# V-Sense/LFBM5D

Measured on AMD Instinct MI355X. Metric: SAI-megapixels/sec (HT+Wiener, sigma=25), higher is better.
Workload: dtype f32; 1 GPU; lf17x17x512x512_sigma25; light_field=17x17x512x512x3, asw=1, color_space=opp, noise=MT19937 seed 1 (utilities.cpp:176-183), window_lanes=2, spatial_bands=1, parallelism=single GPU

## Files before the change

### lfbm5d_amd/core.py

```python
import ctypes as C
import os
import subprocess

from typing import NamedTuple, Optional

import numpy as np

_HERE = os.path.dirname(os.path.abspath(__file__))

YUV, YCBCR, OPP, RGB, ID, DCT, SADCT, BIOR, HADAMARD, HAAR = range(10)
ROWMAJOR, COLMAJOR = 11, 12
TAU = {"id": ID, "dct": DCT, "sadct": SADCT, "bior": BIOR, "hw": HADAMARD, "haar": HAAR}
COLOR_SPACE = {"yuv": YUV, "ycbcr": YCBCR, "opp": OPP, "rgb": RGB}
UNIQUE_ID_BYTES = 128


class LfBm5dError(RuntimeError):
    pass


class Params(C.Structure):
    _fields_ = [("sigma", C.c_float), ("lambda_", C.c_float), ("N", C.c_uint), ("nSim", C.c_uint),
                ("nDisp", C.c_uint), ("k", C.c_uint), ("p", C.c_uint), ("useSD", C.c_uint),
                ("tau_2D", C.c_uint), ("tau_4D", C.c_uint), ("tau_5D", C.c_uint),
# ... 224 lines not shown
    import torch
    if not (isinstance(t, torch.Tensor) and t.is_cuda and t.dtype == torch.float32 and t.is_contiguous()):
        raise LfBm5dError("device entry points need contiguous float32 CUDA tensors")
    torch.cuda.current_stream(t.device).synchronize()
    return C.c_void_p(t.data_ptr())


def _sai_ptrs(arrays, mask):
    out = (C.c_void_p * len(arrays))()
    for i, a in enumerate(arrays):
        if a is None or not mask[i]:
            continue
        if not (isinstance(a, np.ndarray) and a.dtype == np.float32 and a.flags.c_contiguous):
            raise LfBm5dError("per-SAI host buffers must be contiguous float32 numpy arrays")
        out[i] = a.ctypes.data
    return out


OPTION_ENV = ("LFBM5D_LANES", "LFBM5D_EMULATE_WORLD", "LFBM5D_MAX_WINDOWS", "LFBM5D_FUSED", "LFBM5D_STEP_SHARDING",
              "LFBM5D_DATA_DRIVEN_SCHEDULE", "LFBM5D_HOST_BLOCKING", "LFBM5D_BAND_MB", "LFBM5D_BM3D_LANES", "LFBM5D_SCAN_LDS_CAP",
              "LFBM5D_FORCE_REDO", "LFBM5D_SPATIAL_BANDS", "LFBM5D_BAND_HALO", "LFBM5D_SCAN_V1", "LFBM5D_SCAN_ANY", "LFBM5D_SCAN_FULL_TABLES", "LFBM5D_DCT8W_V2",
              "LFBM5D_GROUP_GENERIC", "LFBM5D_NO_SA_KERNELS", "LFBM5D_NO_SLAB_KERNEL", "LFBM5D_WIDE_NOSPLIT", "LFBM5D_AGG_64BIT",
              "LFBM5D_AGG_SCALAR_SCAN", "LFBM5D_SUBSET_LIST_HOST", "LFBM5D_SUBSET_SCAN_V1", "LFBM5D_FILT_GROUP_MAJOR",
              "LFBM5D_HT_REF_ORDER")


class Context:

    def __init__(self, device=0):
        self._L = lib()
        h = C.c_void_p()
        if self._L.lfbm5d_create(C.byref(h), int(device)) != 0:
            raise LfBm5dError(self._L.lfbm5d_last_error(None).decode())
        self._handle = h
        self._env_seen = {k: os.environ.get(k) for k in OPTION_ENV}
        self.device = int(device)

    @property
    def _h(self):
        h = self._handle
        if h and hasattr(self._L, "lfbm5d_set_option"):
            for k in OPTION_ENV:
                v = os.environ.get(k)
                if v != self._env_seen[k]:
                    self._env_seen[k] = v
                    self._L.lfbm5d_set_option(h, k.encode(), None if v is None else (v or "1").encode())
        return h

    def set_option(self, key, value):
        if self._L.lfbm5d_set_option(self._handle, key.encode(), None if value is None else str(value).encode()) != 0:
            raise LfBm5dError(self._L.lfbm5d_last_error(self._handle).decode())

    def get_option(self, key):
        buf = C.create_string_buffer(64)
        if self._L.lfbm5d_get_option(self._handle, key.encode(), buf, 64) != 0:
            raise LfBm5dError(self._L.lfbm5d_last_error(self._handle).decode())
        return buf.value.decode()

    def close(self):
        if getattr(self, "_handle", None):
            self._L.lfbm5d_destroy(self._handle)
            self._handle = None

    def __del__(self):
        try:
            self.close()
        except Exception:
            pass
# ... 246 lines not shown
```

### lfbm5d_amd/csrc/lfbm5d_aggregate.hip

```cpp
#include "lfbm5d_kernels.h"

#include <algorithm>
#include <cstdlib>

namespace lfbm5d {

namespace {



constexpr int kAggFlush = 64;
template <bool WINDOWED, int TW, int TH, int kAggPF, int kAggU, bool BIG, bool VEC4>
__global__ __launch_bounds__(64) __attribute__((amdgpu_waves_per_eu((VEC4 && TW == 8 && !BIG) ? 8 : 1))) void k_aggregate(AggArgs a) {
    constexpr int kAggCap = kAggFlush + kAggPF * 64 + kAggU;
    __shared__ uint4 hit_a[kAggCap];
    __shared__ float hit_w2[kAggCap];
    __shared__ float kai[WINDOWED ? 256 : 1];
    const int lane = threadIdx.x;
    const unsigned gx = (a.Wb + TW - 1) / TW, gy = (a.Hb + TH - 1) / TH, total_wg = gx * gy * a.A;
    const unsigned per_xcd = gridDim.x / 8;
    const unsigned lin2 = (blockIdx.x % 8) * per_xcd + blockIdx.x / 8;
    if (lin2 >= total_wg) return;
    const int st = (int)(lin2 / (gx * gy));
    const int tile_y = (int)((lin2 / gx) % gy), tile_x = (int)(lin2 % gx);
    if (a.proc_bits.test((unsigned)st)) return;
    if (!a.mask_bits.test((unsigned)st)) return;
    const int tx0 = tile_x * TW, ty0 = tile_y * TH;
    const int x = tx0 + lane % TW, y = ty0 + lane / TW;
    const bool inside = x < (int)a.Wb && y < (int)a.Hb;
    const int k = a.k, k2 = k * k, C = a.C, N = a.N, A = a.A;
    const int logN = 31 - __builtin_clz((unsigned)N);
    const size_t plane = (size_t)a.Wb * a.Hb;
    const int reach = (st == (int)a.pst) ? (int)a.nSim : (int)a.nHW;
    if (WINDOWED) for (int i = lane; i < k2; i += 64) kai[i] = a.tb->kaiser[i];

    const int last_r = (int)a.Hb - k - (int)a.nHW, last_c = (int)a.Wb - k - (int)a.nHW;
    auto lo_idx = [&](int v) { int d = v - (int)a.nHW; return d <= 0 ? 0 : (d + (int)a.p - 1) / (int)a.p; };
    auto hi_idx = [&](int v, int n, int lastv) {
        if (v >= lastv) return n - 1;
        int d = v - (int)a.nHW; if (d < 0) return -1;
        int i = d / (int)a.p; return i > n - 2 ? n - 2 : i;
    };
    int r_lo = lo_idx(ty0 - k + 1 - reach), r_hi = hi_idx(ty0 + TH - 1 + reach, (int)a.n_ref_rows, last_r);
    int c_lo = lo_idx(tx0 - k + 1 - reach), c_hi = hi_idx(tx0 + TW - 1 + reach, (int)a.n_ref_cols, last_c);
    if (r_lo > (int)a.n_ref_rows - 1) r_lo = (int)a.n_ref_rows - 1;
    if (c_lo > (int)a.n_ref_cols - 1) c_lo = (int)a.n_ref_cols - 1;
    if (!a.irregular && a.n_ref_cols) {
        r_lo = max(r_lo, (int)(a.ref_begin / a.n_ref_cols));
        r_hi = min(r_hi, (int)((a.ref_begin + a.n_groups - 1) / a.n_ref_cols));
    }
    const int ncols_span = c_hi - c_lo + 1;
    const int n_rr = a.irregular ? (int)a.n_groups : ((r_hi >= r_lo && c_hi >= c_lo) ? (r_hi - r_lo + 1) * ncols_span : 0);
    const int n_cand = n_rr << logN;
    if (n_cand == 0) return;

    float accn[3] = {0, 0, 0}, accd[3] = {0, 0, 0};
    const size_t pix = (size_t)st * C * plane + (size_t)y * a.Wb + x;
    if (inside) for (int c = 0; c < C; c++) { accn[c] = a.num[pix + c * plane]; accd[c] = a.den[pix + c * plane]; }

    const bool mul_div = !a.irregular && (long long)n_rr * ncols_span < (1 << 20);
    const unsigned div_m = ((1u << 20) + (unsigned)max(ncols_span, 1) - 1) / (unsigned)max(ncols_span, 1);
    const unsigned g_end = a.ref_begin + a.n_groups;
    const bool sai_major = a.filt_sai_stride != 0;
    const unsigned Af = sai_major ? 1u : (unsigned)A, stf = sai_major ? 0u : (unsigned)st;
    const float* const filt = a.filt + (sai_major ? (size_t)st * a.filt_sai_stride : (size_t)0);
    const unsigned long long filt_bytes = sai_major ? a.filt_sai_stride * sizeof(float) : a.filt_bytes;
    const bool small24 = (((unsigned long long)a.n_refs_total << logN) + 1) * Af < (1ull << 24);
    const unsigned* apos = a.aggpos + (size_t)st * a.n_refs_total * N;
    const unsigned cstride = C > 1 ? (unsigned)k2 * 4u : 0u;
    const __amdgpu_buffer_rsrc_t rs_filt = __builtin_amdgcn_make_buffer_rsrc((void*)filt, 0, BIG ? 0 : (int)(unsigned)filt_bytes, 0x00020000u);
    unsigned nh = 0;

    auto consume = [&]() {
        const unsigned nh_pad = (nh + kAggU - 1) / kAggU * kAggU;
        if (nh + lane < nh_pad) { hit_a[nh + lane] = make_uint4(0xffffffffu, 0u, 0u, 0u); hit_w2[nh + lane] = 0.0f; }
        __builtin_amdgcn_wave_barrier();
        for (unsigned h0 = 0; h0 < nh_pad; h0 += kAggU) {
            float val[kAggU][3], kw[kAggU][3];
#pragma unroll
            for (int u = 0; u < kAggU; u++) {
// ... 136 lines not shown
                const unsigned slot = nh + __popcll(bal & ((1ull << lane) - 1ull));
                unsigned off;
                const unsigned gl = g[u] - a.ref_begin;
                if (small24) off = __umul24(__umul24((gl << logN) + nn[u], Af) + stf, (unsigned)(C * k2));
                else { asm volatile("" ::: "memory"); off = (((gl << logN) + nn[u]) * Af + stf) * C * k2; }
                hit_a[slot] = make_uint4(p[u], off, __float_as_uint(w[u][0]), __float_as_uint(w[u][1]));
                hit_w2[slot] = w[u][2];
            }
            nh += __popcll(bal);
        }
        __builtin_amdgcn_wave_barrier();
        if (nh >= kAggFlush) consume();
    }
    if (nh) consume();
    if (inside) for (int c = 0; c < C; c++) { a.num[pix + c * plane] = accn[c]; a.den[pix + c * plane] = accd[c]; }
}

}

hipError_t launch_aggregate(hipStream_t s, const AggArgs& a) {
    const bool wide = a.k >= 12;
    constexpr int kAgg16TW = 16, kAgg16TH = 4, kAgg8TW = 8, kAgg8TH = 8;
    const unsigned tw = wide ? (a.k == 12 ? 16 : kAgg16TW) : (a.k == 8 ? kAgg8TW : 8), th = wide ? (a.k == 12 ? 4 : kAgg16TH) : (a.k == 8 ? kAgg8TH : 8);
    const unsigned tiles = ((a.Wb + tw - 1) / tw) * ((a.Hb + th - 1) / th) * a.A;
    const dim3 grid(((tiles + 7) / 8) * 8), block(64);
    const bool big = (a.filt_sai_stride ? a.filt_sai_stride * sizeof(float) : a.filt_bytes) > 0xfffff000ull || (a.opt & kOptAgg64Bit);
    const bool vec4 = a.N % 4 == 0 && !wide && !(a.opt & kOptAggScalarScan);
#define LFBM5D_AGG(W_, TW_, TH_, PF_, U_) \
    do { if (big && vec4) hipLaunchKernelGGL((k_aggregate<W_, TW_, TH_, PF_, U_, true, true>), grid, block, 0, s, a); \
         else if (big)    hipLaunchKernelGGL((k_aggregate<W_, TW_, TH_, PF_, U_, true, false>), grid, block, 0, s, a); \
         else if (vec4)   hipLaunchKernelGGL((k_aggregate<W_, TW_, TH_, PF_, U_, false, true>), grid, block, 0, s, a); \
         else             hipLaunchKernelGGL((k_aggregate<W_, TW_, TH_, PF_, U_, false, false>), grid, block, 0, s, a); } while (0)
    constexpr int kAgg16PF = 3, kAgg16U = 12, kAgg8PF = 3, kAgg8U = 6;
    if (a.k == 12)      LFBM5D_AGG(true, 16, 4, 3, 12);
    else if (a.k == 8)  LFBM5D_AGG(true, kAgg8TW, kAgg8TH, kAgg8PF, kAgg8U);
    else if (wide)      LFBM5D_AGG(false, kAgg16TW, kAgg16TH, kAgg16PF, kAgg16U);
    else                LFBM5D_AGG(false, 8, 8, 2, 6);
#undef LFBM5D_AGG
    return hipGetLastError();
}

}
```

### lfbm5d_amd/csrc/lfbm5d_ctx.h

```cpp
#ifndef LFBM5D_CTX_H
#define LFBM5D_CTX_H

#include "../../include/lfbm5d.h"
#include "lfbm5d_kernels.h"
#include "lfbm5d_plan.h"
#include "lfbm5d_options.h"

#include <rccl/rccl.h>

#include <algorithm>
#include <chrono>
#include <cmath>
#include <fstream>
#include <thread>
#include <unistd.h>
#include <cstdio>
#include <cstdlib>
#include <cstring>
#include <string>
#include <vector>


namespace lfbm5d_host {

// ... 44 lines not shown
    float* const* basic = nullptr;
    float* const* out = nullptr;
};

struct lfbm5d_ctx {
    int device = 0;
    hipStream_t stream = nullptr;
    std::string err;
    int rank = 0, world = 1;
    int tiles = 1;
    ncclComm_t comm = nullptr;
    ncclComm_t comm2 = nullptr;
    hipStream_t cs[2] = {nullptr, nullptr};
    int pass_rank = 0, pass_world = 1;
    bool pass_reduce = false;
    std::vector<unsigned> last_windows;
    lfbm5d_stats stats;
    DevBuf t_noisy, t_basic, t_tnum, t_tden, und_num, und_den;
    DevBuf scan_lcol;
    DevBuf sub_flags, sub_cnt;
    int last_scan_version = 0;
    GeomCache gc[2]; int gslot = 0;
    bool est_ready = false;
    DevBuf est, refmap, scores, tables, self_idx, self_cnt, best, shape, filt, wgt, aggpos, gpos, gofs, gok, sa_list, gshape, counters, small, t_num, t_den, d_mask;
    DevBuf g_num, g_den, g_num2, g_den2, n2, e_basic, w_noisy, w_basic, w_num, w_den, h2d_noisy, h2d_basic, h2d_out, d_own, gscratch;
    bool ipc = false;
    std::string ipc_dir; double ipc_timeout_s = 30.0; unsigned ipc_epoch = 0;
    std::string ipc_tag;
    DevBuf ipc_flags, ipc_out;
    struct IpcPeer { unsigned char handle[7][64]; void* ptr[7]; };
    std::vector<IpcPeer> ipc_peers;
    DevBuf pristine, pristine_b;
    DevBuf band_noisy, band_basic, band_out, band_src, band_pack, band_gather;
    ncclComm_t team_comm = nullptr, team_comm2 = nullptr; int team_S = 0;
    Options opt_store; Options* opt = &opt_store;
    hipStream_t io_in = nullptr, io_out = nullptr;
    unsigned* h_small = nullptr;
    struct NoiseBufs { DevBuf sai, part, cells, m, pool; } noise;
    std::vector<lfbm5d_ctx*> lanes;
    unsigned* h_counts = nullptr; size_t h_counts_cap = 0;
    unsigned long long lane_windows = 0;
    std::vector<hipEvent_t> ev_pool; size_t ev_used = 0;
    std::vector<PassEvents> pending;
    unsigned last_n_refs = 0, last_N = 0, last_A = 0; size_t last_plane = 0; int last_gslot = 0;
};

// ... 45 lines not shown
```

### lfbm5d_amd/csrc/lfbm5d_graph.hip

```cpp
#include "lfbm5d_graph.h"

namespace lfbm5d_host {

using plan::search_window;
using plan::plan_windows;

int io_upload_all(lfbm5d_ctx* c, const HostIO* io, const unsigned* h_mask, unsigned asize, size_t img, float* d_noisy, float* d_basic_in) {
    for (unsigned st = 0; st < asize; st++) {
        if (!h_mask[st]) continue;
        HIPCK(c, hipMemcpyAsync(d_noisy + (size_t)st * img, io->noisy[st], img * sizeof(float), hipMemcpyHostToDevice, c->stream));
        if (d_basic_in) HIPCK(c, hipMemcpyAsync(d_basic_in + (size_t)st * img, io->basic[st], img * sizeof(float), hipMemcpyHostToDevice, c->stream));
    }
    HIPCK(c, hipStreamSynchronize(c->stream));
    return 0;
}
int io_download_all(lfbm5d_ctx* c, const HostIO* io, const unsigned* h_mask, unsigned asize, size_t img, const float* d_noisy,
                    const float* d_basic, const float* d_out) {
    for (unsigned st = 0; st < asize; st++) {
        if (!h_mask[st]) continue;
        HIPCK(c, hipMemcpyAsync(io->noisy[st], d_noisy + (size_t)st * img, img * sizeof(float), hipMemcpyDeviceToHost, c->stream));
        if (d_basic) HIPCK(c, hipMemcpyAsync(io->basic[st], d_basic + (size_t)st * img, img * sizeof(float), hipMemcpyDeviceToHost, c->stream));
        if (d_out) HIPCK(c, hipMemcpyAsync(io->out[st], d_out + (size_t)st * img, img * sizeof(float), hipMemcpyDeviceToHost, c->stream));
    }
    HIPCK(c, hipStreamSynchronize(c->stream));
// ... 58 lines not shown


int run_graph(lfbm5d_ctx* c, const GraphJob& J, const plan::Graph& G, const unsigned* h_mask, unsigned awidth, unsigned aheight,
              unsigned ang_major, unsigned W, unsigned H, unsigned C, int nranks, bool emulate, int* complete_out) {
    const unsigned asize = awidth * aheight;
    const size_t img = (size_t)C * W * H;
    hipStream_t s = c->stream;
    const size_t NN = G.nodes.size();
    const bool two = J.n_steps == 2;
    *complete_out = 1;
    struct Geo { unsigned asw, Aw, nHW, wb, hb; size_t imgb; };
    Geo geo[2];
    size_t imgb_max = 0; unsigned Aw_max = 0;
    for (int sl = 0; sl < J.n_steps; sl++) {
        Geo& g = geo[sl];
        g.asw = 2 * J.an[sl] + 1; g.Aw = g.asw * g.asw; g.nHW = J.P[sl]->nSim + J.P[sl]->nDisp;
        g.wb = W + 2 * g.nHW; g.hb = H + 2 * g.nHW; g.imgb = (size_t)C * g.wb * g.hb;
        imgb_max = std::max(imgb_max, g.Aw * g.imgb); Aw_max = std::max(Aw_max, g.Aw);
    }
    const bool any_step2 = J.step[0] == 2 || (two && J.step[1] == 2);

    struct Lane { lfbm5d_ctx* x; float* w_noisy; float* w_basic; float* w_num; float* w_den; unsigned* d_small; };
    struct RankState { int rank; lfbm5d_ctx* x; float* g_num[2]; float* g_den[2]; float* basic; std::vector<Lane> lanes; };
    auto lane_buffers = [&](lfbm5d_ctx* x, Lane& L) -> int {
        HIPCK(c, x->w_noisy.reserve(imgb_max * sizeof(float)));
        if (any_step2) HIPCK(c, x->w_basic.reserve(imgb_max * sizeof(float)));
        HIPCK(c, x->w_num.reserve(imgb_max * sizeof(float)));
        HIPCK(c, x->w_den.reserve(imgb_max * sizeof(float)));
        HIPCK(c, x->small.reserve((asize + 8 + kWinCounters) * sizeof(unsigned)));
        L.x = x; L.w_noisy = x->w_noisy.as<float>(); L.w_basic = x->w_basic.as<float>();
        L.w_num = x->w_num.as<float>(); L.w_den = x->w_den.as<float>(); L.d_small = x->small.as<unsigned>();
        return 0;
    };
    int lanes_used = 1;
    for (const plan::Node& nd : G.nodes) lanes_used = std::max(lanes_used, nd.lane + 1);
    const int lanes_per_rank = emulate ? 1 : lanes_used;
    const size_t need_ctx = emulate ? (size_t)nranks - 1 : (size_t)lanes_used - 1;
    while (c->lanes.size() < need_ctx) {
        std::string e;
        lfbm5d_ctx* x = new_ctx(c->device, e);
        if (!x) return fail(c, "lane context: " + e);
        x->opt = c->opt;
        c->lanes.push_back(x);
    }
    const bool ipc = c->ipc && nranks > 1 && !emulate;
    struct AbortCommsOnError {
        lfbm5d_ctx* c; bool armed;
        ~AbortCommsOnError() {
            if (!armed) return;
            if (c->comm2) { (void)ncclCommAbort(c->comm2); c->comm2 = nullptr; }
            if (c->comm) { (void)ncclCommAbort(c->comm); c->comm = nullptr; }
            (void)hipDeviceSynchronize();
            c->err += " (multi-GPU step aborted: the RCCL communicators of this context were torn down, call lfbm5d_comm_init again)";
        }
// ... 181 lines not shown
            search_window((int)nd.ps, aheight, J.an[sl], cs_w, mins, maxs);
            search_window((int)nd.pt, awidth, J.an[sl], ct_w, mint, maxt);
            const unsigned cst_w = ang_major == LFBM5D_ROWMAJOR ? (unsigned)cs_w * g.asw + (unsigned)ct_w : (unsigned)cs_w + (unsigned)ct_w * g.asw;
            std::vector<unsigned> mask_w(g.Aw, 0), proc_w(g.Aw, 0);
            SaiList wl; wl.n = g.Aw;
            for (unsigned si = 0; si < g.asw; si++)
                for (unsigned ti = 0; ti < g.asw; ti++) {
                    const unsigned Ss = si + (unsigned)mins, T = ti + (unsigned)mint;
                    const unsigned st = ang_major == LFBM5D_ROWMAJOR ? Ss * awidth + T : Ss + T * aheight;
                    const unsigned slot = ang_major == LFBM5D_ROWMAJOR ? si * g.asw + ti : si + ti * g.asw;
                    mask_w[slot] = h_mask[st];
                    wl.st[slot] = h_mask[st] ? st : 0xffffffffu;
                    if (h_mask[st]) win_bits[n].set(slot);
                    proc_w[slot] = !h_mask[st];
                }
            const bool wien = J.step[sl] == 2;
            HIPCK(c, Lw.x->est.reserve((kEstLead + g.Aw * (size_t)g.wb * g.hb + 256) * sizeof(float)));
            HIPCK(c, launch_window_begin(ls, J.noisy[sl], wien ? S->basic : nullptr, S->g_num[sl], S->g_den[sl], img, Lw.w_noisy, Lw.w_basic, Lw.w_num,
                                         Lw.w_den, Lw.x->est.as<float>() + kEstLead, g.imgb, wl, W, H, C, g.nHW, Lw.d_small));
            lfbm5d_params Pw = *J.P[sl];
            Pw.tau_4D = nd.tau4;
            Lw.x->gslot = sl;
            Lw.x->est_ready = true;
            const int prc = pass_impl(Lw.x, J.step[sl], &Pw, g.asw, g.asw, g.wb, g.hb, C, Lw.w_noisy, wien ? Lw.w_basic : nullptr, Lw.w_num, Lw.w_den,
                                      mask_w.data(), proc_w.data(), cst_w, cst_w);
            Lw.x->gslot = 0;
            if (prc) { if (Lw.x != c) c->err = Lw.x->err; return 1; }
            HIPCK(c, launch_window_end(ls, S->g_num[sl], S->g_den[sl], img, Lw.w_num, Lw.w_den, g.imgb, wl, W, H, C, g.nHW, J.P[sl]->k, Lw.d_small));
            HIPCK(c, hipMemcpyAsync(c->h_counts + (size_t)n * kWinCounters, Lw.d_small, kWinCounters * sizeof(unsigned), hipMemcpyDeviceToHost, ls));
            if (!nd.fin.empty()) {
                SaiList fl; fl.n = 0;
                for (unsigned st : nd.fin) fl.st[fl.n++] = st;
                const bool colour = C == 3 && J.P[0]->color_space != LFBM5D_RGB;
                HIPCK(c, launch_finalize_multi(ls, S->g_num[0], S->g_den[0], J.noisy[0], S->basic, img, fl, J.P[0]->color_space, W * H, colour ? 1 : 0));
            }
            done[n] = get_event(c);
            HIPCK(c, hipEventRecord(done[n], ls));
            mine[n] = 1;
            if (io && !outs[n].empty()) {
                for (size_t o0 = 0; o0 < outs[n].size(); o0 += (size_t)kBigA) {
                    SaiList ol; ol.n = 0;
                    for (size_t q = o0; q < outs[n].size() && ol.n < (unsigned)kBigA; q++) ol.st[ol.n++] = outs[n][q];
                    HIPCK(c, launch_output_multi(ls, S->g_num[Ls], S->g_den[Ls], J.step[Ls] == 1 ? J.noisy[Ls] : S->basic, J.d_out,
                                                 J.step[Ls] == 2 ? S->basic : nullptr, J.noisy[Ls], J.d_noisy, img, ol, J.color_space, W * H, colour_io ? 1 : 0));
                }
                ev_out[n] = get_event(c);
// ... 228 lines not shown
```

### lfbm5d_amd/csrc/lfbm5d_kernels.h

```cpp
#ifndef LFBM5D_KERNELS_H
#define LFBM5D_KERNELS_H

#include <hip/hip_runtime.h>
#include <vector>

#include "lfbm5d_options.h"

constexpr int kFiltStoreAux = 2;
constexpr int kFiltLoadAux = 0;

#if defined(__HIPCC__)
typedef float filt_v4f __attribute__((ext_vector_type(4)));
typedef float filt_v2f __attribute__((ext_vector_type(2)));
__device__ __forceinline__ void filt_put(float* p, const float v) { *p = v; }
__device__ __forceinline__ void filt_put2(filt_v2f* p, const filt_v2f v) { *p = v; }
__device__ __forceinline__ void filt_put4(filt_v4f* p, const filt_v4f v) { *p = v; }
__device__ __forceinline__ void filt_put4(float4* p, const float4 v) { *p = v; }
__device__ __forceinline__ void filt_put4_nt(filt_v4f* p, const filt_v4f v) { __builtin_nontemporal_store(v, p); }
#endif

namespace lfbm5d {

constexpr int kMaxK = 32;
constexpr int kMaxA = 49;
// ... 70 lines not shown
    unsigned Wb, Hb, C, A, k, N, pst;
    SaiMask mask_bits, proc_bits;
    unsigned tau2, tau4, tau5, useSD;
    unsigned fill_quirk;
    int step;
    float lambda;
    float sigma[3];
    float ht3_T[3][9][4];
    float ht3_K[3][9];
    float* scratch;
    unsigned long long scratch_floats;
    unsigned opt;
    unsigned long long filt_sai_stride;
    unsigned bm3d;
};

constexpr unsigned kSaiMajorMinA = 121;
__device__ __forceinline__ size_t filt_patch(const GroupArgs& a, unsigned g, unsigned n, unsigned st, unsigned k2) {
    return a.filt_sai_stride ? (size_t)st * a.filt_sai_stride + ((size_t)g * a.N + n) * a.C * k2
                             : (((size_t)g * a.N + n) * a.A + st) * a.C * k2;
}


struct AggArgs {
    float* num;
    float* den;
    const float* filt;
    unsigned long long filt_sai_stride;
    unsigned long long filt_bytes;
    const float* wgt;
    const unsigned* aggpos;
    unsigned n_refs_total;
    const unsigned* refs;
    const unsigned* self_idx;
    const unsigned* self_cnt;
    const unsigned* best;
    const unsigned char* shape;
    const GroupTables* tb;
    unsigned ref_begin, n_groups;
    unsigned n_ref_rows, n_ref_cols;
    unsigned Wb, Hb, C, A, k, N, pst, p, nHW, nSim, nDisp;
    SaiMask mask_bits, proc_bits; unsigned tau4;
    unsigned irregular;
    unsigned opt;
    unsigned wchan0;
};

__host__ __device__ inline size_t stereo_table_stride(unsigned W, unsigned H, unsigned k, unsigned nDisp) {
    const unsigned ncols = W - 2 * nDisp - (k - 1), nrows = H - 2 * nDisp - (k - 1);
    return (size_t)((ncols + 63) / 64) * 64 * (nrows + 63);
}

__host__ __device__ inline unsigned stereo_table_srq(unsigned H, unsigned k, unsigned nDisp) {
    const unsigned nrows = H - 2 * nDisp - (k - 1);
    return ((nrows - 1 + 63 + 15) / 16) * 4 + 1;
}
__host__ __device__ inline size_t stereo_table_stride2(unsigned W, unsigned H, unsigned k, unsigned nDisp) {
    const unsigned ncols = W - 2 * nDisp - (k - 1);
    return (size_t)((ncols - 1 + 63) / 64) * stereo_table_srq(H, k, nDisp) * 256 + stereo_table_srq(H, k, nDisp) * 4;
}

__host__ __device__ inline unsigned stereo_part_chunks(unsigned H, unsigned k, unsigned nDisp) {
    const unsigned nrows = H - 2 * nDisp - (k - 1);
    return ((nrows - 1 + 63 + 15) / 16) * 2;
}
__host__ __device__ inline size_t stereo_part_stride(unsigned W, unsigned H, unsigned k, unsigned nDisp) {
    const unsigned ncols = W - 2 * nDisp - (k - 1);
    return (size_t)((ncols - 1 + 63) / 64) * stereo_part_chunks(H, k, nDisp) * 512;
// ... 32 lines not shown
    unsigned st_of_slot[kBigA];
    unsigned est_planes;
    const Scan2Wg* wgs;
    unsigned n_wgs;
    float* lcol;
    unsigned lcol_stride;
    unsigned nwg_slot;
};

hipError_t launch_color(hipStream_t s, float* img, unsigned cs, unsigned n_px, int forward);
hipError_t launch_color_lf(hipStream_t s, float* lf, size_t sai_stride, unsigned n_sai, const unsigned* d_mask, unsigned cs,
                           unsigned n_px, int forward);
hipError_t launch_color_roundtrip_lf(hipStream_t s, const float* in, float* out, size_t sai_stride, unsigned n_sai, const unsigned* d_mask,
                                     unsigned cs, unsigned n_px);
hipError_t launch_estimate_lf(hipStream_t s, const float* num, const float* den, const float* sub, float* est, size_t seg,
                              unsigned n_sai, const unsigned* d_mask);
hipError_t launch_symetrize(hipStream_t s, const float* src, float* dst, unsigned W, unsigned H,
                            unsigned C, unsigned N);
hipError_t launch_unsymetrize(hipStream_t s, float* dst, const float* src, unsigned W, unsigned H,
                              unsigned C, unsigned N);
hipError_t launch_crop(hipStream_t s, float* dst, const float* src, unsigned W, unsigned H, unsigned C, unsigned N, unsigned off);
hipError_t launch_estimate(hipStream_t s, const float* num, const float* den, const float* sub,
                           float* est, size_t n);
struct SaiList { unsigned st[kBigA]; unsigned n; };
hipError_t launch_finalize_multi(hipStream_t s, const float* num, const float* den, const float* sub, float* basic, size_t sai_stride,
                                 const SaiList& L, unsigned cs, unsigned n_px, int colour);
hipError_t launch_output_multi(hipStream_t s, const float* num, const float* den, const float* sub, float* out, float* basic,
                               const float* noisy_src, float* noisy_dst, size_t sai_stride, const SaiList& L, unsigned cs, unsigned n_px,
                               int colour);
hipError_t launch_ipc_set(hipStream_t s, unsigned* p, unsigned v);
hipError_t launch_ipc_wait(hipStream_t s, const unsigned* p, unsigned want, unsigned* err, double timeout_s);
hipError_t launch_symetrize_multi(hipStream_t s, const float* src, size_t src_stride, float* dst, size_t dst_stride,
                                  const SaiList& L, unsigned W, unsigned H, unsigned C, unsigned N);
hipError_t launch_unsymetrize_multi(hipStream_t s, float* dst, size_t dst_stride, const float* src, size_t src_stride,
                                    const SaiList& L, unsigned W, unsigned H, unsigned C, unsigned N);
constexpr unsigned kWinCounters = 32;
hipError_t launch_window_begin(hipStream_t s, const float* noisy, const float* basic, const float* num, const float* den, size_t lf_stride,
                               float* w_noisy, float* w_basic, float* w_num, float* w_den, float* est, size_t w_stride, const SaiList& L,
                               unsigned W, unsigned H, unsigned C, unsigned N, unsigned* zero);
hipError_t launch_window_end(hipStream_t s, float* num, float* den, size_t lf_stride, const float* w_num, const float* w_den, size_t w_stride,
                             const SaiList& L, unsigned W, unsigned H, unsigned C, unsigned N, unsigned k, unsigned* count);
hipError_t launch_estimate_multi(hipStream_t s, const float* num, const float* den, const float* sub, float* est,
                                 size_t plane, unsigned C, unsigned A, const SaiMask& mask_bits);
hipError_t launch_copy_rect(hipStream_t s, float* dst, size_t dst_stride, unsigned dW, unsigned dH, unsigned dx0, unsigned dy0,
                            const float* src, size_t src_stride, unsigned sW, unsigned sH, unsigned sx0, unsigned sy0,
                            unsigned w, unsigned h, unsigned C, unsigned n_slots, const SaiMask& mask_bits);
hipError_t launch_copy_rows(hipStream_t s, const float* src, unsigned src_H, unsigned src_row0, float* dst, unsigned dst_H, unsigned dst_row0,
// ... 42 lines not shown
```

### lfbm5d_amd/csrc/lfbm5d_options.h

```cpp
#ifndef LFBM5D_OPTIONS_H
#define LFBM5D_OPTIONS_H

#include <cstddef>
#include <cstdlib>
#include <cstring>
#include <string>

namespace lfbm5d {

enum : unsigned {
    kOptScanV1 = 1u << 0,
    kOptScanAny = 1u << 1,
    kOptScanFullTables = 1u << 2,
    kOptDct8wV2 = 1u << 3,
    kOptGroupGeneric = 1u << 4,
    kOptNoSaKernels = 1u << 5,
    kOptNoSlabKernel = 1u << 6,
    kOptWideNoSplit = 1u << 7,
    kOptAgg64Bit = 1u << 8,
    kOptAggScalarScan = 1u << 9,
    kOptSubsetListHost = 1u << 10,
    kOptSubsetScanV1 = 1u << 11,
    kOptFiltGroupMajor = 1u << 12,
    kOptHtReferenceOrder = 1u << 13,
};

struct Options {
    int lanes = 2;
    int emulate_world = 0;
    int max_windows = 0;
    int fused = 1;
    int step_sharding = 0;
    int data_driven_schedule = 0;
    int host_blocking = 0;
    int band_mb = 0;
    int bm3d_lanes = 3;
    int scan_lds_cap = 0;
    int force_redo = 0;
    int spatial_bands = 1;
    int band_halo = 0;
    unsigned kernels = 0;
};

struct OptionKey { const char* key; const char* env; int Options::* field; unsigned bit; };

inline const OptionKey* option_keys(size_t* n) {
    static const OptionKey keys[] = {
        {"lanes", "LFBM5D_LANES", &Options::lanes, 0}, {"emulate_world", "LFBM5D_EMULATE_WORLD", &Options::emulate_world, 0},
        {"max_windows", "LFBM5D_MAX_WINDOWS", &Options::max_windows, 0}, {"fused", "LFBM5D_FUSED", &Options::fused, 0},
        {"step_sharding", "LFBM5D_STEP_SHARDING", &Options::step_sharding, 0},
        {"data_driven_schedule", "LFBM5D_DATA_DRIVEN_SCHEDULE", &Options::data_driven_schedule, 0},
        {"host_blocking", "LFBM5D_HOST_BLOCKING", &Options::host_blocking, 0}, {"band_mb", "LFBM5D_BAND_MB", &Options::band_mb, 0},
        {"bm3d_lanes", "LFBM5D_BM3D_LANES", &Options::bm3d_lanes, 0}, {"scan_lds_cap", "LFBM5D_SCAN_LDS_CAP", &Options::scan_lds_cap, 0},
        {"force_redo", "LFBM5D_FORCE_REDO", &Options::force_redo, 0}, {"spatial_bands", "LFBM5D_SPATIAL_BANDS", &Options::spatial_bands, 0},
        {"band_halo", "LFBM5D_BAND_HALO", &Options::band_halo, 0},
        {"scan_v1", "LFBM5D_SCAN_V1", nullptr, kOptScanV1}, {"scan_any", "LFBM5D_SCAN_ANY", nullptr, kOptScanAny},
        {"scan_full_tables", "LFBM5D_SCAN_FULL_TABLES", nullptr, kOptScanFullTables}, {"dct8w_v2", "LFBM5D_DCT8W_V2", nullptr, kOptDct8wV2},
        {"group_generic", "LFBM5D_GROUP_GENERIC", nullptr, kOptGroupGeneric}, {"no_sa_kernels", "LFBM5D_NO_SA_KERNELS", nullptr, kOptNoSaKernels},
        {"no_slab_kernel", "LFBM5D_NO_SLAB_KERNEL", nullptr, kOptNoSlabKernel}, {"wide_nosplit", "LFBM5D_WIDE_NOSPLIT", nullptr, kOptWideNoSplit},
        {"agg_64bit", "LFBM5D_AGG_64BIT", nullptr, kOptAgg64Bit}, {"agg_scalar_scan", "LFBM5D_AGG_SCALAR_SCAN", nullptr, kOptAggScalarScan},
        {"subset_list_host", "LFBM5D_SUBSET_LIST_HOST", nullptr, kOptSubsetListHost}, {"subset_scan_v1", "LFBM5D_SUBSET_SCAN_V1", nullptr, kOptSubsetScanV1},
        {"filt_group_major", "LFBM5D_FILT_GROUP_MAJOR", nullptr, kOptFiltGroupMajor},
        {"ht_reference_order", "LFBM5D_HT_REF_ORDER", nullptr, kOptHtReferenceOrder},
    };
    *n = sizeof(keys) / sizeof(keys[0]);
    return keys;
}

inline bool option_set(Options& o, const char* key, const char* value) {
    size_t n; const OptionKey* keys = option_keys(&n);
    static const Options defaults;
    for (size_t i = 0; i < n; i++) {
        if (std::strcmp(key, keys[i].key) != 0 && std::strcmp(key, keys[i].env) != 0) continue;
        const bool unset = value == nullptr || value[0] == 0;
        if (keys[i].field) {
            int v = defaults.*(keys[i].field);
            if (!unset) {
                if (keys[i].field == &Options::step_sharding) v = std::strcmp(value, "rows") == 0 ? 1 : std::strcmp(value, "blocks") == 0 ? 2 : std::atoi(value);
// ... 36 lines not shown
```

### lfbm5d_amd/csrc/lfbm5d_pass.hip

```cpp
#include "lfbm5d_ctx.h"

namespace lfbm5d_host {

lfbm5d_ctx* new_ctx(int device, std::string& err) {
    hipError_t e;
    lfbm5d_ctx* c = new lfbm5d_ctx();
    c->device = device;
    std::memset(&c->stats, 0, sizeof(c->stats));
    if ((e = hipStreamCreateWithFlags(&c->stream, hipStreamNonBlocking)) != hipSuccess) { err = hipGetErrorString(e); delete c; return nullptr; }
    if ((e = prepare_group_kernels()) != hipSuccess || (e = prepare_scan2_kernels()) != hipSuccess) { err = std::string("kernel LDS limits: ") + hipGetErrorString(e); (void)hipStreamDestroy(c->stream); delete c; return nullptr; }
    if ((e = hipHostMalloc((void**)&c->h_small, 64 * sizeof(unsigned))) != hipSuccess) { err = hipGetErrorString(e); (void)hipStreamDestroy(c->stream); delete c; return nullptr; }
    return c;
}


hipEvent_t get_event(lfbm5d_ctx* c) {
    if (c->ev_used == c->ev_pool.size()) {
        hipEvent_t e; (void)hipEventCreate(&e); c->ev_pool.push_back(e);
    }
    return c->ev_pool[c->ev_used++];
}

void drain_events(lfbm5d_ctx* c) {
    for (const PassEvents& pe : c->pending) {
// ... 113 lines not shown
        if (P->nSim < 1 || P->nSim > 48 || P->p < 1) return fail(c, "bad search window / step");
        return 0;
    }
    if (aw != ah || aw < 3 || !(aw & 1) || aw > (unsigned)kBigAw) return fail(c, "unsupported: angular search window must be a square of 3 .. 17 SAIs a side (aswSize 1 to 8)");
    if (C != 1 && C != 3) return fail(c, "unsupported: chnls must be 1 or 3");
    if (P->k < 2 || P->k > (unsigned)kMaxK) return fail(c, "unsupported: patch size k outside 2..32");
    if (P->tau_2D == LFBM5D_BIOR && !is_pow2(P->k)) return fail(c, "bior1.5 needs a power-of-two patch size");
    if (P->tau_2D != LFBM5D_ID && P->tau_2D != LFBM5D_DCT && P->tau_2D != LFBM5D_BIOR) return fail(c, "bad tau_2D");
    if (P->tau_4D != LFBM5D_ID && P->tau_4D != LFBM5D_DCT && P->tau_4D != LFBM5D_SADCT) return fail(c, "bad tau_4D");
    if (P->tau_5D != LFBM5D_HAAR && P->tau_5D != LFBM5D_HADAMARD && P->tau_5D != LFBM5D_DCT) return fail(c, "bad tau_5D");
    if (!is_pow2(P->N) || P->N > (unsigned)kMaxN3) return fail(c, "unsupported: N must be a power of two <= 32");
    if (P->nSim < 1 || P->nDisp < 1 || P->p < 1) return fail(c, "bad search window / step");
    if (P->nSim > 48 || P->nDisp > 24) return fail(c, "unsupported: nSim > 48 or nDisp > 24");
    (void)step;
    return 0;
}

int pass_impl(lfbm5d_ctx* c, int step, const lfbm5d_params* P, unsigned aw, unsigned ah, unsigned Wb,
              unsigned Hb, unsigned C, const float* d_noisy, const float* d_basic, float* d_num,
              float* d_den, const unsigned* h_mask, const unsigned* h_proc, unsigned cst, unsigned pst,
              bool bm3d) {
    const bool est_ready = c->est_ready;
    c->est_ready = false;
    if (validate(c, step, P, aw, ah, C, bm3d)) return 1;
    if (step == 2 && !d_basic) return fail(c, "step 2 needs the basic estimate");
    const unsigned A = aw * ah, k = P->k, k2 = k * k, N = P->N, nHW = P->nSim + P->nDisp;
    const size_t plane = (size_t)Wb * Hb;
    hipStream_t s = c->stream;
    GeomCache& gc = c->gc[c->gslot];
    if (Hb < 2 * nHW + k + 1 || Wb < 2 * nHW + k + 1) return fail(c, "window smaller than the search range");
    if (Hb > 65535 || Wb > 65535) return fail(c, "unsupported: window larger than 65535 pixels a side");

    float sig[3] = {0, 0, 0};
    if (sigma_table(P->sigma, C, P->color_space, sig)) return fail(c, "bad color space");
    const float tauMatch = bm3d ? (step == 1 ? (C == 1 ? 3.f : 1.f) * (sig[0] < 35.0f ? 2500 : 5000)
                                             : (sig[0] < 35.0f ? 400.f : 3500.f))
                                : (C == 1 ? 3.f : 1.f) * (sig[0] < 35.0f ? (step == 1 ? 3000 : 2000) : 5000);
    const float thr = tauMatch * k * k;
    float lambda = P->lambda;
    if (!bm3d && step == 1 && P->tau_2D == LFBM5D_ID && P->tau_4D == LFBM5D_DCT) lambda /= (float)kSqrt2;
    SaiMask mask_bits = sai_mask_none(), proc_bits = sai_mask_none();
    for (unsigned st = 0; st < A; st++) { if (h_mask[st]) mask_bits.set(st); if (h_proc[st]) proc_bits.set(st); }
    if (pst >= A || cst >= A) return fail(c, "cst / pst outside the angular window");
    if (!mask_bits.test(pst)) return fail(c, "processed SAI is empty");

    const bool centre = pst == cst;
    const unsigned key[5] = {Wb, Hb, k, nHW, P->p};
    if (centre && (std::memcmp(key, gc.grid_key, sizeof(key)) != 0 || gc.last_refs_host.empty())) {
        std::vector<unsigned> rows, cols;
        ind_init(rows, Hb - k + 1, nHW, P->p);
        ind_init(cols, Wb - k + 1, nHW, P->p);
        gc.n_ref_rows = (unsigned)rows.size(); gc.n_ref_cols = (unsigned)cols.size();
        gc.last_refs_host.resize(rows.size() * cols.size());
        for (size_t i = 0; i < rows.size(); i++)
            for (size_t j = 0; j < cols.size(); j++) gc.last_refs_host[i * cols.size() + j] = rows[i] * Wb + cols[j];
        std::vector<int> rslot(Hb + 64, -1);
        for (size_t i = 0; i < rows.size(); i++) rslot[rows[i]] = (int)i;
        HIPCK(c, gc.rslot.reserve(rslot.size() * sizeof(int)));
        HIPCK(c, hipMemcpyAsync(gc.rslot.p, rslot.data(), rslot.size() * sizeof(int), hipMemcpyHostToDevice, s));
        HIPCK(c, gc.refs.reserve(gc.last_refs_host.size() * sizeof(unsigned)));
        HIPCK(c, hipMemcpyAsync(gc.refs.p, gc.last_refs_host.data(), gc.last_refs_host.size() * sizeof(unsigned), hipMemcpyHostToDevice, s));
        HIPCK(c, hipStreamSynchronize(s));
        std::memcpy(gc.grid_key, key, sizeof(key));
        std::memcpy(gc.rslot_key, key, sizeof(key));
    }
    unsigned R = gc.n_ref_rows * gc.n_ref_cols;
    const unsigned R_full = R;
    std::vector<unsigned> row_start;
    const bool dev_list = !centre && c->pass_world == 1 && std::memcmp(key, gc.rslot_key, sizeof(key)) == 0 && !(c->opt->kernels & kOptSubsetListHost);
// ... 207 lines not shown
            for (int st = 0; st < 9; st++) {
                double K = 0.0;
                for (int l = 0; l < 4; l++) K = std::max(K, (double)kHtGuardAbs[st][l] / (double)ga.ht3_T[ch][st][l]);
                ga.ht3_K[ch][st] = std::nextafter((float)std::min(K, 1e30), INFINITY);
            }
        }
    }
    ga.bm3d = bm3d ? 1u : 0u;
    ga.opt = c->opt->kernels;
    if (const size_t sb = group_scratch_bytes(ga)) {
        HIPCK(c, c->gscratch.reserve(sb));
        ga.scratch = c->gscratch.as<float>(); ga.scratch_floats = sb / sizeof(float);
    }
    AggArgs aa;
    std::memset(&aa, 0, sizeof(aa));
    aa.num = d_num; aa.den = d_den; aa.wgt = ga.wgt; aa.aggpos = ga.aggpos; aa.n_refs_total = R; aa.refs = ga.refs;
    aa.self_idx = ga.self_idx; aa.self_cnt = ga.self_cnt; aa.best = ga.best; aa.shape = ga.shape; aa.tb = ga.tb;
    aa.ref_begin = ref_begin; aa.n_groups = n_groups; aa.n_ref_rows = gc.n_ref_rows; aa.n_ref_cols = gc.n_ref_cols;
    aa.Wb = Wb; aa.Hb = Hb; aa.C = C; aa.A = A; aa.k = k; aa.N = Nst; aa.pst = pst; aa.p = P->p;
    aa.nHW = nHW; aa.nSim = P->nSim; aa.nDisp = P->nDisp;
    aa.mask_bits = mask_bits; aa.proc_bits = proc_bits; aa.tau4 = P->tau_4D; aa.irregular = centre ? 0u : 1u;
    aa.wchan0 = (bm3d && P->useSD) ? 1u : 0u;
    aa.opt = c->opt->kernels;
    const bool sai_major = A >= kSaiMajorMinA && !(c->opt->kernels & kOptFiltGroupMajor);
    const size_t per_group_bias = sai_major ? per_group / A : per_group;
    if (n_groups <= band_groups) {
        ga.filt_sai_stride = aa.filt_sai_stride = sai_major ? (unsigned long long)n_groups * (per_group / A) : 0ull;
        ga.filt = c->filt.as<float>() - (size_t)ref_begin * per_group_bias;
        aa.filt = c->filt.as<float>(); aa.filt_bytes = (unsigned long long)n_groups * per_group * sizeof(float);
        if (n_groups) HIPCK(c, launch_group(s, ga));
        HIPCK(c, hipEventRecord(pe.e[2], s));
        if (n_groups) HIPCK(c, launch_aggregate(s, aa));
        HIPCK(c, hipEventRecord(pe.e[3], s));
    } else {
        bool first = true;
        for (unsigned b0 = ref_begin; b0 < ref_begin + n_groups; b0 += band_groups) {
            const unsigned nb = std::min(band_groups, ref_begin + n_groups - b0);
            ga.filt_sai_stride = aa.filt_sai_stride = sai_major ? (unsigned long long)nb * (per_group / A) : 0ull;
            ga.ref_begin = b0; ga.n_groups = nb; ga.filt = c->filt.as<float>() - (size_t)b0 * per_group_bias;
            aa.ref_begin = b0; aa.n_groups = nb; aa.filt = c->filt.as<float>(); aa.filt_bytes = (unsigned long long)nb * per_group * sizeof(float);
            HIPCK(c, launch_group(s, ga));
            if (first) HIPCK(c, hipEventRecord(pe.e[2], s));
            first = false;
            HIPCK(c, launch_aggregate(s, aa));
            c->stats.launches_group += 1; c->stats.launches_aggregate += 1;
        }
// ... 46 lines not shown
```

### lfbm5d_amd/csrc/lfbm5d_window.hip

```cpp
#include "lfbm5d_kernels.h"

#include <algorithm>

namespace lfbm5d {

namespace {


__device__ __forceinline__ void color_px(unsigned cs, int fwd, const float R, const float G, const float B, float& x, float& y, float& z) {
#pragma clang fp contract(off)
    if (cs == 0) {
        if (fwd) { x = 0.299f * R + 0.587f * G + 0.114f * B; y = -0.14713f * R - 0.28886f * G + 0.436f * B; z = 0.615f * R - 0.51498f * G - 0.10001f * B; }
        else     { x = R + 1.13983f * B; y = R - 0.39465f * G - 0.5806f * B; z = R + 2.03211f * G; }
    } else if (cs == 1) {
        if (fwd) { x = 0.299f * R + 0.587f * G + 0.114f * B; y = -0.169f * R - 0.331f * G + 0.500f * B; z = 0.500f * R - 0.419f * G - 0.081f * B; }
        else     { x = 1.000f * R + 0.000f * G + 1.402f * B; y = 1.000f * R - 0.344f * G - 0.714f * B; z = 1.000f * R + 1.772f * G + 0.000f * B; }
    } else {
        if (fwd) { x = 0.333f * R + 0.333f * G + 0.333f * B; y = 0.500f * R + 0.000f * G - 0.500f * B; z = 0.250f * R - 0.500f * G + 0.250f * B; }
        else     { x = 1.0f * R + 1.0f * G + 0.666f * B; y = 1.0f * R + 0.0f * G - 1.333f * B; z = 1.0f * R - 1.0f * G + 0.666f * B; }
    }
}

__global__ void k_color(float* __restrict__ img, size_t sai_stride, const unsigned* __restrict__ mask, unsigned cs, unsigned n, int fwd) {
    const unsigned i = blockIdx.x * blockDim.x + threadIdx.x;
// ... 221 lines not shown
    if (threadIdx.x == 0 && t) atomicAdd(count, t);
}

struct WinBeginArgs {
    const float* noisy; const float* basic; const float* num; const float* den;
    float* w_noisy; float* w_basic; float* w_num; float* w_den;
    float* est;
    size_t lf_stride, w_stride;
    SaiList L;
    int W, H, C, N;
    unsigned* zero;
};
__global__ __launch_bounds__(256) void k_window_begin(WinBeginArgs a) {
    if (blockIdx.x == 0 && blockIdx.y == 0 && blockIdx.z == 0 && threadIdx.y == 0 && threadIdx.x < kWinCounters && a.zero) a.zero[threadIdx.x] = 0u;
    const unsigned st = a.L.st[blockIdx.z];
    if (st == 0xffffffffu) return;
    const int w = a.W + 2 * a.N, h = a.H + 2 * a.N;
    const int xx = blockIdx.x * 64 + threadIdx.x, yy = blockIdx.y * 4 + threadIdx.y;
    if (xx >= w || yy >= h) return;
    const size_t so = (size_t)st * a.lf_stride + (size_t)mirror(yy - a.N, a.H) * a.W + mirror(xx - a.N, a.W);
    const size_t d_o = (size_t)blockIdx.z * a.w_stride + (size_t)yy * w + xx;
    const size_t sp = (size_t)a.W * a.H, dp = (size_t)w * h;
    float n0 = 0.0f, u0 = 0.0f, d0 = 0.0f, b0 = 0.0f;
    for (int c = 0; c < a.C; c++) {
        const float nv = a.noisy[so + c * sp], uv = a.num[so + c * sp], dv = a.den[so + c * sp];
        a.w_noisy[d_o + c * dp] = nv; a.w_num[d_o + c * dp] = uv; a.w_den[d_o + c * dp] = dv;
        float bv = 0.0f;
        if (a.basic) { bv = a.basic[so + c * sp]; a.w_basic[d_o + c * dp] = bv; }
        if (c == 0) { n0 = nv; u0 = uv; d0 = dv; b0 = bv; }
    }
    a.est[(size_t)blockIdx.z * dp + (size_t)yy * w + xx] = d0 ? __fdiv_rn(u0, d0) : (a.basic ? b0 : n0);
}

struct WinEndArgs {
    float* num; float* den; const float* w_num; const float* w_den;
    size_t lf_stride, w_stride;
    SaiList L;
    int W, H, C, N, k;
    unsigned* count;
};
constexpr int kWinEndRows = 32;
static_assert(kWinCounters == 32, "k_window_end");
constexpr int kWinEndCounters = 32;
__global__ __launch_bounds__(256) void k_window_end(WinEndArgs a) {
    __shared__ unsigned red[4];
    const unsigned st = a.L.st[blockIdx.z];
    if (st == 0xffffffffu) return;
    const int w = a.W + 2 * a.N, h = a.H + 2 * a.N;
    const int x = blockIdx.x * 64 + threadIdx.x;
    const size_t dp = (size_t)a.W * a.H, sp = (size_t)w * h;
    unsigned cnt = 0;
    if (x < a.W)
        for (int r = 0; r < kWinEndRows; r += 4) {
            const int y = blockIdx.y * kWinEndRows + r + threadIdx.y;
            if (y >= a.H) break;
            const size_t d_o = (size_t)st * a.lf_stride + (size_t)y * a.W + x;
            const size_t so = (size_t)blockIdx.z * a.w_stride + (size_t)(y + a.N) * w + x + a.N;
            const bool counted = x < a.W - a.k + 1 && y < a.H - a.k + 1;
            for (int c = 0; c < a.C; c++) {
                const float dv = a.w_den[so + c * sp];
                a.num[d_o + c * dp] = a.w_num[so + c * sp];
                a.den[d_o + c * dp] = dv;
                cnt += (counted && dv > 0.0f) ? 1u : 0u;
            }
        }
    for (int o = 32; o > 0; o >>= 1) cnt += __shfl_xor(cnt, o);
    if (threadIdx.x == 0) red[threadIdx.y] = cnt;
    __syncthreads();
    if (threadIdx.x == 0 && threadIdx.y == 0) {
        const unsigned t = red[0] + red[1] + red[2] + red[3];
        if (t) atomicAdd(a.count + (blockIdx.x + blockIdx.y * 5 + blockIdx.z * 11) % kWinEndCounters, t);
    }
}

}


static inline dim3 grid1d(size_t n, unsigned b = 256) { return dim3((unsigned)((n + b - 1) / b)); }

hipError_t launch_color(hipStream_t s, float* img, unsigned cs, unsigned n_px, int forward) {
    hipLaunchKernelGGL(k_color, grid1d(n_px), dim3(256), 0, s, img, (size_t)0, (const unsigned*)nullptr, cs, n_px, forward);
// ... 130 lines not shown
```

Baseline: 240.8 SAI-megapixels/s.

## Aggregate directly into global light-field sums instead of padded window copies

By default the aggregation kernel now reads and writes numerator and denominator sums in place in the global per-SAI light-field buffers, offset by the window padding. This removes the padded w_num/w_den window buffers, their copy-in in k_window_begin, and their copy-back in k_window_end, which now only counts covered pixels. It adds SAI-index indirection and the lf_stride argument to the aggregation kernel and limits the direct path to single-world graph windows. The old padded path stays available behind an option.

```diff
diff --git a/lfbm5d_amd/core.py b/lfbm5d_amd/core.py
--- a/lfbm5d_amd/core.py
+++ b/lfbm5d_amd/core.py
@@ -270,7 +270,8 @@
               "LFBM5D_FORCE_REDO", "LFBM5D_SPATIAL_BANDS", "LFBM5D_BAND_HALO", "LFBM5D_SCAN_V1", "LFBM5D_SCAN_ANY", "LFBM5D_SCAN_FULL_TABLES", "LFBM5D_DCT8W_V2",
               "LFBM5D_GROUP_GENERIC", "LFBM5D_NO_SA_KERNELS", "LFBM5D_NO_SLAB_KERNEL", "LFBM5D_WIDE_NOSPLIT", "LFBM5D_AGG_64BIT",
               "LFBM5D_AGG_SCALAR_SCAN", "LFBM5D_SUBSET_LIST_HOST", "LFBM5D_SUBSET_SCAN_V1", "LFBM5D_FILT_GROUP_MAJOR",
-              "LFBM5D_HT_REF_ORDER")
+              "LFBM5D_HT_REF_ORDER", "LFBM5D_WINDOW_SUMS_PADDED")
+OPTION_ENV_EMPTY_OFF = ("LFBM5D_WINDOW_SUMS_PADDED",)
 
 
 class Context:
@@ -292,6 +293,8 @@
                 v = os.environ.get(k)
                 if v != self._env_seen[k]:
                     self._env_seen[k] = v
+                    if not v and k in OPTION_ENV_EMPTY_OFF:
+                        v = None
                     self._L.lfbm5d_set_option(h, k.encode(), None if v is None else (v or "1").encode())
         return h
 
diff --git a/lfbm5d_amd/csrc/lfbm5d_aggregate.hip b/lfbm5d_amd/csrc/lfbm5d_aggregate.hip
--- a/lfbm5d_amd/csrc/lfbm5d_aggregate.hip
+++ b/lfbm5d_amd/csrc/lfbm5d_aggregate.hip
@@ -17,7 +17,8 @@
     __shared__ float hit_w2[kAggCap];
     __shared__ float kai[WINDOWED ? 256 : 1];
     const int lane = threadIdx.x;
-    const unsigned gx = (a.Wb + TW - 1) / TW, gy = (a.Hb + TH - 1) / TH, total_wg = gx * gy * a.A;
+    const unsigned org = a.direct ? a.nHW : 0u, Wt = a.Wb - 2 * org, Ht = a.Hb - 2 * org;
+    const unsigned gx = (Wt + TW - 1) / TW, gy = (Ht + TH - 1) / TH, total_wg = gx * gy * a.A;
     const unsigned per_xcd = gridDim.x / 8;
     const unsigned lin2 = (blockIdx.x % 8) * per_xcd + blockIdx.x / 8;
     if (lin2 >= total_wg) return;
@@ -25,12 +26,12 @@
     const int tile_y = (int)((lin2 / gx) % gy), tile_x = (int)(lin2 % gx);
     if (a.proc_bits.test((unsigned)st)) return;
     if (!a.mask_bits.test((unsigned)st)) return;
-    const int tx0 = tile_x * TW, ty0 = tile_y * TH;
+    const int tx0 = (int)org + tile_x * TW, ty0 = (int)org + tile_y * TH;
     const int x = tx0 + lane % TW, y = ty0 + lane / TW;
-    const bool inside = x < (int)a.Wb && y < (int)a.Hb;
+    const bool inside = x < (int)(org + Wt) && y < (int)(org + Ht);
     const int k = a.k, k2 = k * k, C = a.C, N = a.N, A = a.A;
     const int logN = 31 - __builtin_clz((unsigned)N);
-    const size_t plane = (size_t)a.Wb * a.Hb;
+    const size_t plane = (size_t)Wt * Ht;
     const int reach = (st == (int)a.pst) ? (int)a.nSim : (int)a.nHW;
     if (WINDOWED) for (int i = lane; i < k2; i += 64) kai[i] = a.tb->kaiser[i];
 
@@ -55,7 +56,7 @@
     if (n_cand == 0) return;
 
     float accn[3] = {0, 0, 0}, accd[3] = {0, 0, 0};
-    const size_t pix = (size_t)st * C * plane + (size_t)y * a.Wb + x;
+    const size_t pix = (a.direct ? (size_t)a.sai.st[st] * a.lf_stride : (size_t)st * C * plane) + (size_t)(y - (int)org) * Wt + (size_t)(x - (int)org);
     if (inside) for (int c = 0; c < C; c++) { accn[c] = a.num[pix + c * plane]; accd[c] = a.den[pix + c * plane]; }
 
     const bool mul_div = !a.irregular && (long long)n_rr * ncols_span < (1 << 20);
@@ -238,7 +239,8 @@
     const bool wide = a.k >= 12;
     constexpr int kAgg16TW = 16, kAgg16TH = 4, kAgg8TW = 8, kAgg8TH = 8;
     const unsigned tw = wide ? (a.k == 12 ? 16 : kAgg16TW) : (a.k == 8 ? kAgg8TW : 8), th = wide ? (a.k == 12 ? 4 : kAgg16TH) : (a.k == 8 ? kAgg8TH : 8);
-    const unsigned tiles = ((a.Wb + tw - 1) / tw) * ((a.Hb + th - 1) / th) * a.A;
+    const unsigned org = a.direct ? a.nHW : 0u;
+    const unsigned tiles = ((a.Wb - 2 * org + tw - 1) / tw) * ((a.Hb - 2 * org + th - 1) / th) * a.A;
     const dim3 grid(((tiles + 7) / 8) * 8), block(64);
     const bool big = (a.filt_sai_stride ? a.filt_sai_stride * sizeof(float) : a.filt_bytes) > 0xfffff000ull || (a.opt & kOptAgg64Bit);
     const bool vec4 = a.N % 4 == 0 && !wide && !(a.opt & kOptAggScalarScan);
diff --git a/lfbm5d_amd/csrc/lfbm5d_ctx.h b/lfbm5d_amd/csrc/lfbm5d_ctx.h
--- a/lfbm5d_amd/csrc/lfbm5d_ctx.h
+++ b/lfbm5d_amd/csrc/lfbm5d_ctx.h
@@ -90,6 +90,7 @@
     int last_scan_version = 0;
     GeomCache gc[2]; int gslot = 0;
     bool est_ready = false;
+    struct DirectSums { bool on = false; float* num = nullptr; float* den = nullptr; size_t lf_stride = 0; lfbm5d::SaiList sai; } direct;
     DevBuf est, refmap, scores, tables, self_idx, self_cnt, best, shape, filt, wgt, aggpos, gpos, gofs, gok, sa_list, gshape, counters, small, t_num, t_den, d_mask;
     DevBuf g_num, g_den, g_num2, g_den2, n2, e_basic, w_noisy, w_basic, w_num, w_den, h2d_noisy, h2d_basic, h2d_out, d_own, gscratch;
     bool ipc = false;
diff --git a/lfbm5d_amd/csrc/lfbm5d_graph.hip b/lfbm5d_amd/csrc/lfbm5d_graph.hip
--- a/lfbm5d_amd/csrc/lfbm5d_graph.hip
+++ b/lfbm5d_amd/csrc/lfbm5d_graph.hip
@@ -104,14 +104,17 @@
 
     struct Lane { lfbm5d_ctx* x; float* w_noisy; float* w_basic; float* w_num; float* w_den; unsigned* d_small; };
     struct RankState { int rank; lfbm5d_ctx* x; float* g_num[2]; float* g_den[2]; float* basic; std::vector<Lane> lanes; };
+    const bool direct = !c->opt->window_sums_padded;
     auto lane_buffers = [&](lfbm5d_ctx* x, Lane& L) -> int {
         HIPCK(c, x->w_noisy.reserve(imgb_max * sizeof(float)));
         if (any_step2) HIPCK(c, x->w_basic.reserve(imgb_max * sizeof(float)));
-        HIPCK(c, x->w_num.reserve(imgb_max * sizeof(float)));
-        HIPCK(c, x->w_den.reserve(imgb_max * sizeof(float)));
+        if (!direct) {
+            HIPCK(c, x->w_num.reserve(imgb_max * sizeof(float)));
+            HIPCK(c, x->w_den.reserve(imgb_max * sizeof(float)));
+        }
         HIPCK(c, x->small.reserve((asize + 8 + kWinCounters) * sizeof(unsigned)));
         L.x = x; L.w_noisy = x->w_noisy.as<float>(); L.w_basic = x->w_basic.as<float>();
-        L.w_num = x->w_num.as<float>(); L.w_den = x->w_den.as<float>(); L.d_small = x->small.as<unsigned>();
+        L.w_num = direct ? nullptr : x->w_num.as<float>(); L.w_den = direct ? nullptr : x->w_den.as<float>(); L.d_small = x->small.as<unsigned>();
         return 0;
     };
     int lanes_used = 1;
@@ -339,6 +342,7 @@
             Pw.tau_4D = nd.tau4;
             Lw.x->gslot = sl;
             Lw.x->est_ready = true;
+            if (direct) { Lw.x->direct.on = true; Lw.x->direct.num = S->g_num[sl]; Lw.x->direct.den = S->g_den[sl]; Lw.x->direct.lf_stride = img; Lw.x->direct.sai = wl; }
             const int prc = pass_impl(Lw.x, J.step[sl], &Pw, g.asw, g.asw, g.wb, g.hb, C, Lw.w_noisy, wien ? Lw.w_basic : nullptr, Lw.w_num, Lw.w_den,
                                       mask_w.data(), proc_w.data(), cst_w, cst_w);
             Lw.x->gslot = 0;
diff --git a/lfbm5d_amd/csrc/lfbm5d_kernels.h b/lfbm5d_amd/csrc/lfbm5d_kernels.h
--- a/lfbm5d_amd/csrc/lfbm5d_kernels.h
+++ b/lfbm5d_amd/csrc/lfbm5d_kernels.h
@@ -116,6 +116,8 @@
 }
 
 
+struct SaiList { unsigned st[kBigA]; unsigned n; };
+
 struct AggArgs {
     float* num;
     float* den;
@@ -138,6 +140,9 @@
     unsigned irregular;
     unsigned opt;
     unsigned wchan0;
+    unsigned direct;
+    unsigned long long lf_stride;
+    SaiList sai;
 };
 
 __host__ __device__ inline size_t stereo_table_stride(unsigned W, unsigned H, unsigned k, unsigned nDisp) {
@@ -216,7 +221,6 @@
 hipError_t launch_crop(hipStream_t s, float* dst, const float* src, unsigned W, unsigned H, unsigned C, unsigned N, unsigned off);
 hipError_t launch_estimate(hipStream_t s, const float* num, const float* den, const float* sub,
                            float* est, size_t n);
-struct SaiList { unsigned st[kBigA]; unsigned n; };
 hipError_t launch_finalize_multi(hipStream_t s, const float* num, const float* den, const float* sub, float* basic, size_t sai_stride,
                                  const SaiList& L, unsigned cs, unsigned n_px, int colour);
 hipError_t launch_output_multi(hipStream_t s, const float* num, const float* den, const float* sub, float* out, float* basic,
diff --git a/lfbm5d_amd/csrc/lfbm5d_options.h b/lfbm5d_amd/csrc/lfbm5d_options.h
--- a/lfbm5d_amd/csrc/lfbm5d_options.h
+++ b/lfbm5d_amd/csrc/lfbm5d_options.h
@@ -39,6 +39,7 @@
     int force_redo = 0;
     int spatial_bands = 1;
     int band_halo = 0;
+    int window_sums_padded = 0;
     unsigned kernels = 0;
 };
 
@@ -54,6 +55,7 @@
         {"bm3d_lanes", "LFBM5D_BM3D_LANES", &Options::bm3d_lanes, 0}, {"scan_lds_cap", "LFBM5D_SCAN_LDS_CAP", &Options::scan_lds_cap, 0},
         {"force_redo", "LFBM5D_FORCE_REDO", &Options::force_redo, 0}, {"spatial_bands", "LFBM5D_SPATIAL_BANDS", &Options::spatial_bands, 0},
         {"band_halo", "LFBM5D_BAND_HALO", &Options::band_halo, 0},
+        {"window_sums_padded", "LFBM5D_WINDOW_SUMS_PADDED", &Options::window_sums_padded, 0},
         {"scan_v1", "LFBM5D_SCAN_V1", nullptr, kOptScanV1}, {"scan_any", "LFBM5D_SCAN_ANY", nullptr, kOptScanAny},
         {"scan_full_tables", "LFBM5D_SCAN_FULL_TABLES", nullptr, kOptScanFullTables}, {"dct8w_v2", "LFBM5D_DCT8W_V2", nullptr, kOptDct8wV2},
         {"group_generic", "LFBM5D_GROUP_GENERIC", nullptr, kOptGroupGeneric}, {"no_sa_kernels", "LFBM5D_NO_SA_KERNELS", nullptr, kOptNoSaKernels},
diff --git a/lfbm5d_amd/csrc/lfbm5d_pass.hip b/lfbm5d_amd/csrc/lfbm5d_pass.hip
--- a/lfbm5d_amd/csrc/lfbm5d_pass.hip
+++ b/lfbm5d_amd/csrc/lfbm5d_pass.hip
@@ -159,6 +159,8 @@
               bool bm3d) {
     const bool est_ready = c->est_ready;
     c->est_ready = false;
+    const bool direct = c->direct.on;
+    c->direct.on = false;
     if (validate(c, step, P, aw, ah, C, bm3d)) return 1;
     if (step == 2 && !d_basic) return fail(c, "step 2 needs the basic estimate");
     const unsigned A = aw * ah, k = P->k, k2 = k * k, N = P->N, nHW = P->nSim + P->nDisp;
@@ -182,6 +184,7 @@
     if (!mask_bits.test(pst)) return fail(c, "processed SAI is empty");
 
     const bool centre = pst == cst;
+    if (direct && (!centre || !est_ready || bm3d || c->pass_world != 1 || c->pass_reduce)) return fail(c, "direct sums: not a single-pass window of the graph form");
     const unsigned key[5] = {Wb, Hb, k, nHW, P->p};
     if (centre && (std::memcmp(key, gc.grid_key, sizeof(key)) != 0 || gc.last_refs_host.empty())) {
         std::vector<unsigned> rows, cols;
@@ -435,6 +438,9 @@
     aa.mask_bits = mask_bits; aa.proc_bits = proc_bits; aa.tau4 = P->tau_4D; aa.irregular = centre ? 0u : 1u;
     aa.wchan0 = (bm3d && P->useSD) ? 1u : 0u;
     aa.opt = c->opt->kernels;
+    if (direct) {
+        aa.num = c->direct.num; aa.den = c->direct.den; aa.direct = 1u; aa.lf_stride = c->direct.lf_stride; aa.sai = c->direct.sai;
+    }
     const bool sai_major = A >= kSaiMajorMinA && !(c->opt->kernels & kOptFiltGroupMajor);
     const size_t per_group_bias = sai_major ? per_group / A : per_group;
     if (n_groups <= band_groups) {
diff --git a/lfbm5d_amd/csrc/lfbm5d_window.hip b/lfbm5d_amd/csrc/lfbm5d_window.hip
--- a/lfbm5d_amd/csrc/lfbm5d_window.hip
+++ b/lfbm5d_amd/csrc/lfbm5d_window.hip
@@ -267,9 +267,13 @@
     const size_t d_o = (size_t)blockIdx.z * a.w_stride + (size_t)yy * w + xx;
     const size_t sp = (size_t)a.W * a.H, dp = (size_t)w * h;
     float n0 = 0.0f, u0 = 0.0f, d0 = 0.0f, b0 = 0.0f;
+    const bool sums = a.w_num != nullptr;
     for (int c = 0; c < a.C; c++) {
-        const float nv = a.noisy[so + c * sp], uv = a.num[so + c * sp], dv = a.den[so + c * sp];
-        a.w_noisy[d_o + c * dp] = nv; a.w_num[d_o + c * dp] = uv; a.w_den[d_o + c * dp] = dv;
+        const float nv = a.noisy[so + c * sp];
+        float uv = 0.0f, dv = 0.0f;
+        if (sums || c == 0) { uv = a.num[so + c * sp]; dv = a.den[so + c * sp]; }
+        a.w_noisy[d_o + c * dp] = nv;
+        if (sums) { a.w_num[d_o + c * dp] = uv; a.w_den[d_o + c * dp] = dv; }
         float bv = 0.0f;
         if (a.basic) { bv = a.basic[so + c * sp]; a.w_basic[d_o + c * dp] = bv; }
         if (c == 0) { n0 = nv; u0 = uv; d0 = dv; b0 = bv; }
@@ -302,6 +306,10 @@
             const size_t d_o = (size_t)st * a.lf_stride + (size_t)y * a.W + x;
             const size_t so = (size_t)blockIdx.z * a.w_stride + (size_t)(y + a.N) * w + x + a.N;
             const bool counted = x < a.W - a.k + 1 && y < a.H - a.k + 1;
+            if (!a.w_den) {
+                if (counted) for (int c = 0; c < a.C; c++) cnt += a.den[d_o + c * dp] > 0.0f ? 1u : 0u;
+                continue;
+            }
             for (int c = 0; c < a.C; c++) {
                 const float dv = a.w_den[so + c * sp];
                 a.num[d_o + c * dp] = a.w_num[so + c * sp];
```

Result: faster. 246.6 SAI-megapixels/s (median of 6 runs) (+2.4%).
